# jfjlaros/HUMID

Hardware: AMD Instinct MI355X
Metric: reads/sec deduplicated, 10M PE150 UMI=8 d=1 (higher is better)
Workload: dtype u64; 1 GPU; 10000000 reads/GPU x 1 GPU (one shuffled read set of 10000000 reads, sliced by input order), PE150 UMI=8 in header -> 24-nt packed words (8+8+8), d=1, directional clustering; synthetic molecules=N/4, family 1+Geom(3), p_sub=1e-3, p_N=1e-4; reads_per_gpu=10000000, word_nt=24, distance=1, method=directional

## Files before the change

### humid_amd/_lib.py

```python
from __future__ import annotations

import ctypes as C
import os

_HERE = os.path.dirname(os.path.abspath(__file__))
SO_PATH = os.path.join(_HERE, "libhumid_hip.so")

u64p = C.POINTER(C.c_uint64)
u32p = C.POINTER(C.c_uint32)
u8p = C.POINTER(C.c_uint8)


class HumidSummary(C.Structure):
    _fields_ = [("total", C.c_uint64), ("usable", C.c_uint64), ("unique", C.c_uint64),
                ("clusters", C.c_uint64), ("edges", C.c_uint64), ("nonsingle", C.c_uint64),
                ("ms_count", C.c_float), ("ms_neighbours", C.c_float), ("ms_cluster", C.c_float),
                ("ms_map", C.c_float), ("ms_total", C.c_float), ("ms_h2d", C.c_float),
                ("ms_d2h", C.c_float), ("ms_k_insert", C.c_float), ("ms_k_pairs", C.c_float),
                ("ms_k_cluster", C.c_float), ("ms_k_map", C.c_float), ("ms_k_part", C.c_float),
                ("ms_k_unperm", C.c_float), ("count_mode_used", C.c_uint32)]

    def asdict(self):
        d = {k: getattr(self, k) for k, _ in self._fields_}
        d["records8"] = bool(d["count_mode_used"] >> 8)
# ... 209 lines not shown
                                    C.c_uint64, C.c_uint64, C.c_uint64, u64p, u64p]),
    "humid_stage_unique": (C.c_int, [C.c_void_p, C.POINTER(C.c_void_p), C.POINTER(C.c_void_p),
                                     C.POINTER(C.c_void_p)]),
    "humid_stage_graph": (C.c_int, [C.c_void_p, C.c_void_p, C.c_void_p, C.c_uint64, C.c_uint32,
                                    C.c_uint32, C.c_uint32, C.POINTER(C.c_void_p),
                                    C.POINTER(C.c_void_p), C.POINTER(HumidSummary)]),
    "humid_stage_map": (C.c_int, [C.c_void_p, C.c_void_p, C.c_void_p, C.c_uint64, C.c_void_p,
                                  C.c_void_p]),
    "humid_stage_count_dense": (C.c_int, [C.c_void_p, C.c_void_p, C.c_void_p, C.c_uint64, C.c_uint32,
                                          C.c_uint64, C.c_uint64, u64p, C.c_uint32, u64p, u64p, u64p]),
    "humid_stage_map_dense": (C.c_int, [C.c_void_p, C.c_void_p, C.c_void_p, C.POINTER(C.c_void_p), u64p]),
    "humid_stage_pairs": (C.c_int, [C.c_void_p, C.c_void_p, C.c_uint64, C.c_uint32, C.c_uint32,
                                    C.c_uint32, C.c_uint32, C.POINTER(C.c_void_p), u64p]),
    "humid_graph_split_info": (C.c_int, [C.c_void_p, C.POINTER(C.c_uint64), C.POINTER(C.c_uint64), u32p]),
    "humid_group_records_info": (C.c_int, [C.c_void_p, u32p, u32p]),
    "humid_get_run_roads": (C.c_int, [C.c_void_p, C.POINTER(HumidRunRoads)]),
    "humid_stage_kernel_ms": (C.c_int, [C.c_void_p, C.POINTER(C.c_float), C.POINTER(C.c_float), u32p]),
    "humid_stage_route_words": (C.c_int, [C.c_void_p, C.c_void_p, C.c_uint64, C.POINTER(C.c_void_p)]),
    "humid_stage_route": (C.c_int, [C.c_void_p, C.c_void_p, C.c_void_p, C.c_uint64, u64p, u64p, C.c_uint32, u64p,
                                    C.POINTER(C.c_void_p), C.POINTER(C.c_void_p)]),
    "humid_stage_route_check": (C.c_int, [C.c_void_p]),
    "humid_stage_exchange_ids": (C.c_int, [C.c_void_p, C.c_void_p, C.c_void_p, C.c_void_p, C.c_uint64,
                                           C.c_uint64, C.c_uint64, C.c_uint64, C.POINTER(C.c_void_p),
                                           C.POINTER(C.c_void_p)]),
    "humid_stage_plan_info": (C.c_int, [C.c_void_p, C.c_uint32, C.c_uint32, C.c_uint64, u32p, u32p]),
    "humid_stage_combo_route": (C.c_int, [C.c_void_p, C.c_void_p, C.c_void_p, C.c_uint64, C.c_uint64,
                                          C.c_uint32, C.c_uint32, C.c_uint64, C.c_uint32, C.c_uint32,
                                          C.POINTER(C.c_void_p), u64p]),
    "humid_stage_pairs_keyed": (C.c_int, [C.c_void_p, C.c_void_p, C.c_uint64, C.c_int, C.c_uint64,
                                          C.c_void_p, C.c_uint32, C.c_uint32, C.c_uint64, C.c_uint32,
# ... 66 lines not shown
```

### humid_amd/api.py

```python
from __future__ import annotations

import ctypes as C

import numpy as np

from . import _lib

DIRECTIONAL = 0
MAXIMUM = 1

BEST_LEAF, BEST_CLUSTER = 0, 1
NO_READ = 0xffffffff
NO_TILE = 0xffffffff
_BEST_SCOPES = {"leaf": BEST_LEAF, "cluster": BEST_CLUSTER, BEST_LEAF: BEST_LEAF, BEST_CLUSTER: BEST_CLUSTER}

STRAND_TOP, STRAND_BOTTOM, STRAND_NONE = 0, 1, 2

BC_FILTERED, BC_EXACT, BC_CORRECTED, BC_AMBIGUOUS, BC_UNMATCHED = range(5)

CELLS_TOP, CELLS_EXPECTED, CELLS_MIN_READS = 0, 1, 2


class HumidError(RuntimeError):
    def __init__(self, code, msg):
# ... 621 lines not shown
            self._check(self._lib.humid_get_leaf_groups(self._h, _vp(out["group"])))
        if getattr(self, "_keyed_summary", None) is self.summary:
            out["key"] = self.group_keys()[out["group"]] if u else np.zeros(0, np.uint64)
        return out

    def graph_split_info(self):
        a, b, f = C.c_uint64(), C.c_uint64(), C.c_uint32()
        self._check(self._lib.humid_graph_split_info(self._h, C.byref(a), C.byref(b), C.byref(f)))
        return dict(pairs_direct=a.value, pairs_graph=b.value, full_graph_built=f.value)

    def group_records_info(self):
        a, b = C.c_uint32(), C.c_uint32()
        self._check(self._lib.humid_group_records_info(self._h, C.byref(a), C.byref(b)))
        return dict(searched_on_records=a.value, orders_stored=b.value)

    def run_roads(self):
        r = _lib.HumidRunRoads()
        self._check(self._lib.humid_get_run_roads(self._h, C.byref(r)))
        return r.asdict()

    def adjacency(self):
        u = int(self.summary["unique"])
        e2 = 2 * int(self.summary["edges"])
        off = np.zeros(u + 1, np.uint32)
        idx = np.zeros(max(e2, 1), np.uint32)
        self._check(self._lib.humid_get_adjacency(self._h, _vp(off), _vp(idx)))
        return off, idx[:e2]

    def clusters(self):
        c = int(self.summary["clusters"])
# ... 218 lines not shown
```

### humid_amd/csrc/humid_hip.hip

```cpp
#include "pipeline.hip.h"
#include "passes.hip.h"

static std::string g_err;
extern "C" __attribute__((visibility("hidden"))) void humid_set_global_error(const char *text) { g_err = text ? text : ""; }

extern "C" {

uint32_t humid_abi_version(void) { return HUMID_ABI_VERSION; }

int humid_device_count(void) {
  int n = 0;
  if (hipGetDeviceCount(&n) != hipSuccess) return 0;
  return n;
}

const char *humid_last_error(const humid_ctx *ctx) { return ctx ? ctx->err.c_str() : g_err.c_str(); }

int humid_ctx_create(humid_ctx **out, int device, void *stream) {
  humid_ctx *c = nullptr;
  if (!out) return fail(nullptr, HUMID_E_INVALID, "out is null");
  *out = nullptr;
  int ndev = 0;
  hipError_t e = hipGetDeviceCount(&ndev);
  if (e != hipSuccess || ndev == 0)
// ... 146 lines not shown
  }
  if (strcmp(key, "group_buckets") == 0) {
    c->group_buckets = value != 0;
    return HUMID_OK;
  }
  if (strcmp(key, "fused_search") == 0) {
    c->fused_search = value != 0;
    return HUMID_OK;
  }
  if (strcmp(key, "pair_split") == 0) {
    c->pair_split = value != 0;
    return HUMID_OK;
  }
  if (strcmp(key, "group_records") == 0) {
    c->group_records = value != 0;
    return HUMID_OK;
  }
  if (strcmp(key, "padded_partition") == 0) {
    c->pt_padded = value != 0;
    return HUMID_OK;
  }
  if (strcmp(key, "force_comm") == 0) {
    c->force_comm = value != 0;
    return HUMID_OK;
  }
  if (strcmp(key, "bucket_walk") == 0) {
    if (value < 0 || value > (1 << 24)) return fail(c, HUMID_E_INVALID, "bucket_walk must be 0 (no limit) .. 2^24");
    c->walk_max = (u32)value;
    return HUMID_OK;
  }
// ... 239 lines not shown
int humid_graph_split_info(humid_ctx *c, uint64_t *pairs_direct, uint64_t *pairs_graph, uint32_t *full_graph_built) {
  if (!c) return fail(nullptr, HUMID_E_INVALID, "ctx is null");
  if (!state_has_leaves(c)) return fail(c, HUMID_E_STATE, "no completed dedup run / graph stage in this context");
  const bool split = c->cg_valid && c->cg_split;
  if (pairs_direct) *pairs_direct = split ? c->cg_iso : 0;
  if (pairs_graph) *pairs_graph = split ? c->cg_R : c->E;
  if (full_graph_built) *full_graph_built = (!split || c->cg_full) ? 1u : 0u;
  return HUMID_OK;
}

int humid_group_records_info(humid_ctx *c, uint32_t *searched_on_records, uint32_t *orders_stored) {
  if (!c) return fail(nullptr, HUMID_E_INVALID, "ctx is null");
  if (!state_has_leaves(c)) return fail(c, HUMID_E_STATE, "no completed dedup run / graph stage in this context");
  if (searched_on_records) *searched_on_records = c->cg_valid ? c->gr_rides : 0u;
  if (orders_stored) *orders_stored = c->cg_valid ? c->gr_orders : 0u;
  return HUMID_OK;
}

int humid_get_run_roads(humid_ctx *c, humid_run_roads *out) {
  if (!c) return fail(nullptr, HUMID_E_INVALID, "ctx is null");
  if (!out) return fail(c, HUMID_E_INVALID, "null argument");
  if (c->state.holds == CtxState::NOTHING) return fail(c, HUMID_E_STATE, "no completed run or stage call in this context");
  *out = c->roads;
  return HUMID_OK;
}

int humid_get_leaves(humid_ctx *c, uint64_t *word, uint32_t *count, uint32_t *first_read,
                     uint32_t *degree, uint32_t *cluster_id, uint8_t *is_max_leaf) {
  NEED_LEAVES();
  size_t U = (size_t)c->gU;
// ... 1167 lines not shown
```

### humid_amd/csrc/kernels_part8.hip.h

```cpp
#ifndef HUMID_KERNELS_PART8_HIP_H
#define HUMID_KERNELS_PART8_HIP_H

#include "common.hip.h"
#include "kernels_count.hip.h"
#include "kernels_part.hip.h"

#define P8_CAP2_LOG 10u
#define P8_CAP2 (1u << P8_CAP2_LOG)
#define P8_RPT (P8_CAP2 / 256u)

struct RecKey {
  u64 lo, scale;
  u32 z, kbits;
  u32 pow2;
  __host__ __device__ __forceinline__ u64 operator()(u64 w) const { return ((w - lo) * scale) >> z; }
  __device__ __forceinline__ u64 word(u64 k) const {
    if (pow2) return lo + k;
    const u64 x = k << z, q = x / scale;
    return lo + q + ((x - q * scale) ? 1u : 0u);
  }
};

struct Reads8 {
  const u64 *words;
// ... 70 lines not shown
    goff[threadIdx.x] = threadIdx.x * cap1 + (had < cap1 ? had : cap1);
    if (had + c > cap1) ctr[OVER] = 1;
  }
  PH(5);
#pragma unroll
  for (u32 q = 0; q < PT_IPT; q++)
    if (binrank[q] != NONE32) srec[loff[binrank[q] >> 16] + (binrank[q] & 0xffffu)] = rec[q];
  __syncthreads();
  PH(6);
  p8_write_bins(srec, loff, nb, p8_group(loff[nb], nb), out,
                [&](u32 bin, u32 k) -> u64 { return goff[bin] + k < (bin + 1) * cap1 ? (u64)goff[bin] + k : ~0ull; });
  PH(7);
  PH_END(1, 7, (blockIdx.x & 15u) == 3u);
}

static __global__ void __launch_bounds__(1024, 8)
k_p8_scatter2(const u64 *__restrict__ in, const u32 *__restrict__ tprefix, const u32 *__restrict__ cbase, u32 kbits, u32 d1,
              u32 d2, u32 ibits, u32 cap1, u32 *cursor2, u64 *__restrict__ out, ull *ctr) {
  HUMID_GUARD_LAST_VGPR();
  __shared__ u64 srec[PT_TILE];
  __shared__ u32 cnt[PT_MAXBINS], loff[PT_MAXBINS + 1], goff[PT_MAXBINS], room[PT_MAXBINS], wsum[8];
  __shared__ u32 s_c, s_beg, s_cnt;
  PH_DECL;
  PH(0);
  if (blockIdx.x >= tprefix[1u << d1]) return;
  const u32 nb = 1u << d2;
  if (threadIdx.x == 0) {
    u32 c, b, n;
    pt_tile_of(tprefix, cbase, 1u << d1, blockIdx.x, cap1, c, b, n);
    s_c = c; s_beg = b; s_cnt = n;
  }
  for (u32 b = threadIdx.x; b < nb; b += PT_THREADS) cnt[b] = 0;
  __syncthreads();
  PH(1);
  const u32 coarse = s_c, t_beg = s_beg, t_cnt = s_cnt;
  const u32 fshift = ibits + kbits - d1 - d2;
  u64 rec[PT_IPT];
  u32 binrank[PT_IPT];
#pragma unroll
  for (u32 q = 0; q < PT_IPT; q++) {
    const u32 j = threadIdx.x + q * PT_THREADS;
    binrank[q] = NONE32;
    if (j < t_cnt) rec[q] = in[t_beg + j];
  }
#pragma unroll
  for (u32 q = 0; q < PT_IPT; q++) {
    const u32 j = threadIdx.x + q * PT_THREADS;
    if (j < t_cnt) {
      const u32 bin = (u32)(rec[q] >> fshift) & (nb - 1);
      binrank[q] = bin << 16 | atomicAdd(&cnt[bin], 1u);
// ... 519 lines not shown
```

### humid_amd/csrc/pipeline.hip.h

```cpp
#ifndef HUMID_PIPELINE_HIP_H
#define HUMID_PIPELINE_HIP_H

#include <fcntl.h>
#include <sys/mman.h>
#include <sys/stat.h>
#include <unistd.h>

#include <atomic>
#include <cerrno>
#include <chrono>
#include <type_traits>
#include <utility>

#include "common.hip.h"
#include "prims.hip.h"
#include "kernels_count.hip.h"
#include "kernels_part.hip.h"
#include "kernels_part8.hip.h"
#include "kernels_graph.hip.h"
#include "kernels_cluster.hip.h"
#include "kernels_cgraph.hip.h"
#include "kernels_map.hip.h"
#include "kernels_xchg.hip.h"
#include "kernels_wide.hip.h"
// ... 127 lines not shown
  const u32 *ctr_x[3] = {nullptr, nullptr, nullptr};
  DBuf xo_gw, xo_gc;
  DBuf xo_regs, xo_inv;
  u64 xr_ecap = 0;
  DBuf xo_send, xo_int, xo_cross, xo_sel, xo_selall, xo_parent, xo_flag, xo_xroot, xo_xcbits, xo_xcblk, xo_xcid, xo_xcall, xo_ldeg, xo_cnt;
  DBuf pw_a, pw_ai, pw_b, pw_bi;
  DBuf p8_a, p8_b, p8_cur, p8_status;
  bool use_rec8 = true;
  bool last_rec8 = false;
  const u32 *rec_cursor2 = nullptr;
  DBuf pt_work, unperm_rec, route_tiles;
  bool group_buckets = true;
  bool fused_search = true;
  bool group_records = true;
  u32 gr_rides = 0, gr_orders = 0;
  bool pt_padded = true;
  bool use_tile_partition = true;
  bool last_part_tiled = false;
  int x_test_fail_after = -1, x_gathers = 0;
  bool x_hist_done = false, x_peer_failed = false;
  bool route_checked = true;
  const u32 *route_bad = nullptr;
  bool last_unperm_tiled = false;
  bool oc_valid = false, oc_fits = false;
  u32 oc_n = 0, oc_nt = 0;
  u64 oc_lo = 0, oc_scale = 0;
  u32 n_parts = 0;
  bool stage_map_timed = false;
  bool last_count_sorted = false;
  u32 g_wpr = 1;
// ... 166 lines not shown
  }
  __threadfence_system();
  __syncthreads();
  if (threadIdx.x == 0) { host[CTR_N] = seq; __threadfence_system(); }
}
static int read_counters_begin(humid_ctx *c, const u32 *extra32 = nullptr, const u32 *extra32b = nullptr, const u32 *extra32c = nullptr) {
  c->ctr_x[0] = extra32; c->ctr_x[1] = extra32b; c->ctr_x[2] = extra32c;
  if (c->h_ctr_dev && !c->no_poll) {
    const ull seq = ++c->ctr_seq;
    hipLaunchKernelGGL(k_publish_counters, dim3(1), dim3(64), 0, c->stream, (const ull *)c->d_ctr, extra32, extra32b,
                       (volatile ull *)c->h_ctr_dev, seq, extra32c);
    HIPCHK(hipGetLastError());
  }
  return HUMID_OK;
}
static int read_counters_end(humid_ctx *c) {
  const u32 *extra32 = c->ctr_x[0], *extra32b = c->ctr_x[1], *extra32c = c->ctr_x[2];
  if (c->h_ctr_dev && !c->no_poll) {
    const ull seq = c->ctr_seq;
    volatile ull *flag = (volatile ull *)&c->h_ctr[CTR_N];
    const auto t0 = std::chrono::steady_clock::now();
    u32 spins = 0;
    while (*flag != seq) {
      if ((++spins & 0xfffu) == 0) {
        if (hipStreamQuery(c->stream) != hipErrorNotReady) break;
        if (std::chrono::steady_clock::now() - t0 > std::chrono::seconds(30)) break;
      }
    }
    if (*flag == seq) { std::atomic_thread_fence(std::memory_order_acquire); return HUMID_OK; }
    HIPCHK(hipStreamSynchronize(c->stream));
    if (*flag == seq) return HUMID_OK;
    c->no_poll = true;
// ... 12 lines not shown
static int read_counters(humid_ctx *c, const u32 *extra32 = nullptr, const u32 *extra32b = nullptr, const u32 *extra32c = nullptr) {
  const int rc = read_counters_begin(c, extra32, extra32b, extra32c);
  return rc != HUMID_OK ? rc : read_counters_end(c);
}

#define TRY(...) do { int _rc = (__VA_ARGS__); if (_rc != HUMID_OK) return _rc; } while (0)

static int scan_total(humid_ctx *c, const u32 *in, u32 *out, u64 n, u64 *total) {
  TRY(exscan_u32(c, in, out, n + 1));
  HIPCHK(hipGetLastError());
  TRY(read_counters(c, out + n));
  *total = c->h_ctr[CTR_N - 1] & 0xffffffffull;
  return HUMID_OK;
}

static inline void state_reset(humid_ctx *c) { c->state = CtxState{}; c->roads = humid_run_roads{}; }
static inline void road_taken(humid_ctx *c, u8 road) {
  if (c->roads.n_events < HUMID_ROADS_MAX) c->roads.events[c->roads.n_events] = road;
  c->roads.n_events++;
}
static inline void state_begin_graph(humid_ctx *c) { const bool dense = c->state.dense; state_reset(c); c->state.dense = dense; }
static inline int state_publish(humid_ctx *c, CtxState::Holds holds) {
  const bool dense = holds == CtxState::STAGE_GRAPH && c->state.dense;
  c->state = CtxState{holds, holds == CtxState::RUN ? c->pass_kind : RUN_PLAIN, dense, false};
  return HUMID_OK;
}
static inline int state_publish_count(humid_ctx *c, bool dense) { state_publish(c, CtxState::COUNT); c->state.dense = dense; return HUMID_OK; }
static inline bool state_has_leaves(const humid_ctx *c) { return c->state.holds == CtxState::RUN || c->state.holds == CtxState::STAGE_GRAPH; }
static inline bool state_has_run(const humid_ctx *c) { return c->state.holds == CtxState::RUN; }
static inline bool state_dense_count(const humid_ctx *c) { return c->state.dense; }
static inline bool state_run_is(const humid_ctx *c, RunKind at_least) { return state_has_run(c) && c->state.kind >= at_least; }
// ... 109 lines not shown
    hipLaunchKernelGGL(k_cluster_trivial<true>, dim3(blocks_for(U)), dim3(256), 0, st, g.deg, g.parent, g.csize, U, g_cnt, g.off,
                       g.idx, g.cl_of, g.maxleaf, g.cl_size);
  else
    hipLaunchKernelGGL(k_cluster_trivial<false>, dim3(blocks_for(U)), dim3(256), 0, st, g.deg, g.parent, g.csize, U, g_cnt, g.off,
                       g.idx, g.cl_of, g.maxleaf, g.cl_size);
  if (M > 0) {
    const u64 small_cap = M / 3 + 1;
    if (late_m) TRY(read_counters_begin(c, nullptr, nullptr, late_m));
    if (method == HUMID_METHOD_MAXIMUM)
      hipLaunchKernelGGL(k_cluster_small_lds<true>, dim3(blocks_for(small_cap, 64)), dim3(64), 0, st, c->small_roots.as<u32>(),
                         (const ull *)c->d_ctr, g.parent, g.csize, U, g_cnt, g.off, g.idx, g.cl_of, g.maxleaf, g.cl_size);
    else
      hipLaunchKernelGGL(k_cluster_small_lds<false>, dim3(blocks_for(small_cap, 64)), dim3(64), 0, st, c->small_roots.as<u32>(),
                         (const ull *)c->d_ctr, g.parent, g.csize, U, g_cnt, g.off, g.idx, g.cl_of, g.maxleaf, g.cl_size);
    if (late_m) {
      TRY(read_counters_end(c));
      Mbig = c->h_ctr[CTR_MEMBERS];
      M = c->h_ctr[CTR_N - 3] & 0xffffffffull;
      U = (u32)M;
      if (late_m_out) *late_m_out = M;
    }
    if (Mbig > 0) {
      ENSURE(c->mk0, (size_t)Mbig * 8);
      ENSURE(c->mk1, (size_t)Mbig * 8);
      ENSURE(c->stk, (size_t)Mbig * 8);
      HIPCHK(hipMemsetAsync(&c->d_ctr[CTR_SPECIAL], 0, sizeof(ull), st));
      hipLaunchKernelGGL(k_member_keys, dim3(COMPACT_BLOCKS), dim3(256), 0, st, g.deg, g.parent, g.csize, U, c->mk0.as<u64>(), c->d_ctr);
      TRY(sort_keys<u64>(c, c->mk0.as<u64>(), c->mk1.as<u64>(), Mbig, 0, 32 + bits_for(U)));
      if (method == HUMID_METHOD_MAXIMUM) {
        hipLaunchKernelGGL(k_cluster_components<true>, dim3(blocks_for(Mbig, 64)), dim3(64), 0, st,
                           c->mk1.as<u64>(), (u32)Mbig, g_cnt, g.off, g.idx, g.cl_of, g.maxleaf, g.cl_size, c->stk.as<u32>());
// ... 311 lines not shown
    z.p[0] = cursor1; z.n[0] = PT_MAXBINS1 + n_parts;
    z.p[1] = (u32 *)c->d_ctr; z.n[1] = 2 * CTR_N;
    z.p[2] = (u32 *)(agg + n_parts); z.n[2] = 2;
    hipLaunchKernelGGL(k_zero_many, dim3(32), dim3(256), 0, st, z);
  }
  const bool check_range = !(range_lo == 0 && range_hi == ~0ull);
  const Reads8 src{d_words, d_filt, range_lo, range_hi, check_range ? 1u : 0u, rk};
  const u32 tiles1 = (N + PT_TILE - 1) / PT_TILE, tiles2 = tiles1 + nb1;
  static const bool s1_small = getenv("HUMID_S1_THREADS") ? atoi(getenv("HUMID_S1_THREADS")) == 512 : false;
  if (s1_small && nb1 <= 512)
    hipLaunchKernelGGL((k_p8_scatter1<Reads8, 512>), dim3((N + 4095) / 4096), dim3(512), 0, st, src, N, rk.kbits, d1, ibits, cap1, cursor1,
                       c->p8_a.as<u64>(), c->d_ctr);
  else
    hipLaunchKernelGGL((k_p8_scatter1<Reads8, 1024>), dim3(tiles1), dim3(1024), 0, st, src, N, rk.kbits, d1, ibits, cap1, cursor1,
                       c->p8_a.as<u64>(), c->d_ctr);
  hipLaunchKernelGGL(k_pt_scan1, dim3(1), dim3(1024), 0, st, (const u32 *)cursor1, d1, d2, cbase, tprefix, c->pbeg.as<u32>(),
                     c->ucount.as<u32>() + n_parts, cap1);
  if (c->kev_on) HIPCHK(hipEventRecord(c->kev[39], st));
  hipLaunchKernelGGL(k_p8_scatter2, dim3(tiles2), dim3(1024), 0, st, (const u64 *)c->p8_a.as<u64>(), (const u32 *)tprefix,
                     (const u32 *)cbase, rk.kbits, d1, d2, ibits, cap1, cursor2, c->p8_b.as<u64>(), c->d_ctr);
  if (c->kev_on) HIPCHK(hipEventRecord(c->kev[40], st));
  HIPCHK(hipEventRecord(c->kev[0], st));
  hipLaunchKernelGGL(k_dedup_rec, dim3(n_parts), dim3(256), 0, st, c->p8_b.as<u64>(), (const u32 *)cursor2, N, pb, d1, ibits, rk,
                     c->pad_word.as<u64>(), c->pad_cf.as<uint2>(), agg, c->d_ctr);
  HIPCHK(hipEventRecord(c->kev[1], st));
  TRY(exscan_in<u64>(c, PtrIn<u64>{agg}, abase, (u64)n_parts + 1));
  ENSURE(c->s_word, (size_t)(N + 1) * 8);
  ENSURE(c->s_slot, (size_t)(N + 1) * 4);
  ENSURE(c->s_cnt, (size_t)(N + 1) * 4);
  ENSURE(c->s_first, (size_t)(N + 1) * 4);
  hipLaunchKernelGGL(k_compact_padded8, dim3(blocks_for((u64)n_parts * 64)), dim3(256), 0, st, c->pad_word.as<u64>(),
                     c->pad_cf.as<uint2>(), (const u64 *)agg, (const u64 *)abase, n_parts, c->s_word.as<u64>(),
                     c->s_slot.as<u32>(), c->s_cnt.as<u32>(), c->s_first.as<u32>());
  if (!c->lean_events) HIPCHK(hipEventRecord(c->ev[1], st));
  HIPCHK(hipGetLastError());
  TRY(read_counters(c, (const u32 *)(abase + n_parts), (const u32 *)(abase + n_parts) + 1));
  if (getenv("HUMID_TRACE_COUNT"))
    fprintf(stderr, "[rec count] N %u pb %u kbits %u ibits %u cap1 %u special %llu overfull %llu unique %llu usable %llu\n", N, pb, rk.kbits,
            ibits, cap1, (ull)c->h_ctr[CTR_SPECIAL], (ull)c->h_ctr[CTR_OVERFULL], (ull)(c->h_ctr[CTR_N - 1] & 0xffffffffull), (ull)(c->h_ctr[CTR_N - 2] & 0xffffffffull));
  if (c->h_ctr[CTR_SPECIAL]) { c->pt_padded = false; road_taken(c, HUMID_ROAD_PART_PADDED_REDO); return HUMID_OK; }
  if (c->h_ctr[CTR_OVERFULL]) return HUMID_OK;
  c->last_count_lds = true;
  c->last_count_sorted = false;
  c->last_count_ordered = true;
  c->last_part_tiled = true;
  c->last_rec8 = true;
  c->rec_cursor2 = cursor2;
  c->n_parts = n_parts;
  const u32 U = (u32)(c->h_ctr[CTR_N - 1] & 0xffffffffull);
  s.usable = c->usable = c->h_ctr[CTR_N - 2] & 0xffffffffull;
  s.unique = c->U = U;
// ... 55 lines not shown
  if (c->kev_on) HIPCHK(hipEventRecord(c->kev[40], st));
  HIPCHK(hipEventRecord(c->kev[0], st));
  hipLaunchKernelGGL((k_dedup_wide_rec<9, 512, 0, WL_SMALL_LEN>), dim3(n_parts), dim3(256), 0, st, (const W2 *)c->pw_b.as<W2>(),
                     (const u32 *)c->pw_bi.as<u32>(), (const u32 *)cursor2, hbits, rk, N, pb, c->pad_word.as<W2>(), c->pad_cf.as<uint2>(),
                     agg, c->p8_b.as<u64>(), c->d_ctr);
  if (N > WL_SMALL_LEN)
    hipLaunchKernelGGL((k_dedup_wide_rec<10, 1024, WL_SMALL_LEN, WL_STAGE>), dim3(n_parts), dim3(256), 0, st,
                       (const W2 *)c->pw_b.as<W2>(), (const u32 *)c->pw_bi.as<u32>(), (const u32 *)cursor2, hbits, rk, N, pb,
                       c->pad_word.as<W2>(), c->pad_cf.as<uint2>(), agg, c->p8_b.as<u64>(), c->d_ctr);
  HIPCHK(hipEventRecord(c->kev[1], st));
  TRY(exscan_in<u64>(c, PtrIn<u64>{agg}, abase, (u64)n_parts + 1));
  ENSURE(c->s_word, (size_t)(N + 1) * 16);
  ENSURE(c->s_slot, (size_t)(N + 1) * 4);
  ENSURE(c->s_cnt, (size_t)(N + 1) * 4);
  ENSURE(c->s_first, (size_t)(N + 1) * 4);
  hipLaunchKernelGGL(k_compact_padded8_wide, dim3(blocks_for((u64)n_parts * 64)), dim3(256), 0, st, (const W2 *)c->pad_word.as<W2>(),
                     (const uint2 *)c->pad_cf.as<uint2>(), (const u64 *)agg, (const u64 *)abase, n_parts, c->s_word.as<W2>(),
                     c->s_slot.as<u32>(), c->s_cnt.as<u32>(), c->s_first.as<u32>());
  if (!c->lean_events) HIPCHK(hipEventRecord(c->ev[1], st));
  HIPCHK(hipGetLastError());
  TRY(read_counters(c, (const u32 *)(abase + n_parts), (const u32 *)(abase + n_parts) + 1));
  if (getenv("HUMID_TRACE_COUNT"))
    fprintf(stderr, "[rec count, wide] N %u pb %u kbits %u cap1 %u special %llu overfull %llu unique %llu usable %llu\n", N, pb, rk.kbits, cap1,
            (ull)c->h_ctr[CTR_SPECIAL], (ull)c->h_ctr[CTR_OVERFULL], (ull)(c->h_ctr[CTR_N - 1] & 0xffffffffull), (ull)(c->h_ctr[CTR_N - 2] & 0xffffffffull));
  if (c->h_ctr[CTR_SPECIAL] || c->h_ctr[CTR_OVERFULL]) return HUMID_OK;
  c->last_count_lds = true;
  c->last_count_sorted = false;
  c->last_count_ordered = true;
  c->last_part_tiled = true;
  c->last_rec8 = true;
  c->rec_cursor2 = cursor2;
  c->n_parts = n_parts;
  const u32 U = (u32)(c->h_ctr[CTR_N - 1] & 0xffffffffull);
  s.usable = c->usable = c->h_ctr[CTR_N - 2] & 0xffffffffull;
  s.unique = c->U = U;
  *done = true;
// ... 587 lines not shown
  const u32 *cnt_by_id;
  u32 n_ids;
  u64 pairs_bound;
  u32 *bits = nullptr;
  bool no_wait = false;
};
struct CgStatus {
  bool overflow = false;
  bool group_over = false;
  u64 wanted = 0, big_mask = 0, E = 0, M = 0, Mbig = 0;
};
static GraphArrays cg_arrays(humid_ctx *c) {
  return GraphArrays{c->cg_deg.as<u32>(), c->cg_parent.as<u32>(), c->cg_csize.as<u32>(), c->cg_off.as<u32>(), c->cg_idx.as<u32>(),
                     c->cg_cl_of.as<u32>(), c->cg_maxleaf.as<u32>(), c->cg_cl_size.as<u64>()};
}
static int cg_build(humid_ctx *c, CgSource &src, u32 method, CgStatus &out) {
  hipStream_t st = c->stream;
  u32 *bits = src.bits ? src.bits : c->cg_bits.as<u32>();
  const u32 n_words = (((src.n_ids + 31) / 32) + 7) & ~7u, n_blk = n_words / 8;
  const u64 pb = std::max<u64>(src.pairs_bound, 1);
  if (2 * pb + 2 > 0xffffffffull) return fail(c, HUMID_E_OVERFLOW, "too many neighbour pairs");
  const u32 Mb = (u32)std::min<u64>(src.n_ids, 2 * pb);
  ENSURE(c->cg_blk, ((size_t)n_blk + 1) * 4);
  ENSURE(c->cg_nodes, ((size_t)Mb + 1) * 4);
  ENSURE(c->cg_ncnt, ((size_t)Mb + 1) * 4);
  ENSURE(c->cg_deg, ((size_t)Mb + 2) * 4);
  ENSURE(c->cg_off, ((size_t)Mb + 2) * 4);
  ENSURE(c->cg_parent, ((size_t)Mb + 1) * 4);
  ENSURE(c->cg_csize, ((size_t)Mb + 1) * 4);
  ENSURE(c->cg_curs, ((size_t)Mb + 1) * 4);
  ENSURE(c->cg_idx, (size_t)(2 * pb + 1) * 4);
  ENSURE(c->cg_cl_of, ((size_t)Mb + 1) * 4);
  ENSURE(c->cg_maxleaf, ((size_t)Mb + 1) * 4);
  ENSURE(c->cg_cl_size, ((size_t)Mb + 1) * 8);
  ENSURE(c->small_roots, ((size_t)Mb / 3 + 2) * 4);
  ENSURE(c->small, 64);
  TRY(exscan_in<u32>(c, BitsBlockIn{bits, n_blk}, c->cg_blk.as<u32>(), (u64)n_blk + 1));
  const BitRank br{bits, c->cg_blk.as<u32>()};
  const u32 *m_dev = c->cg_blk.as<u32>() + n_blk;
  const GraphArrays g = cg_arrays(c);
  const u32 r_first = src.er.e ? 0u : ER_REGIONS;
  hipLaunchKernelGGL(k_nodes_init, dim3(blocks_for(n_words)), dim3(256), 0, st, br, n_words, src.cnt_by_id, c->cg_nodes.as<u32>(),
                     c->cg_ncnt.as<u32>(), g.deg, g.parent, g.csize, c->cg_curs.as<u32>(), n_blk);
  const bool by_count = (method & 1) == 0;
  if (src.segs) {
    const u32 n_all = src.segs->first[REC_SEGS];
    u32 n_max = 1;
    for (u32 q = 0; q < REC_SEGS; q++) n_max = std::max(n_max, src.segs->n[q]);
    ENSURE(c->cg_far, ((size_t)n_all + 1) * 8);
    hipLaunchKernelGGL(k_segs_relabel, dim3(std::min<u32>(blocks_for(n_max), 4096), REC_SEGS), dim3(256), 0, st, *src.segs, src.n_ids, br,
                       c->cg_far.as<u64>(), c->cg_ncnt.as<u32>(), g.deg, g.parent, by_count);
    src.er.far = c->cg_far.as<u64>();
    src.er.n_far = n_all;
  } else if (src.recs) {
    ENSURE(c->cg_far, ((size_t)src.n_recs + 1) * 8);
    if (src.n_recs)
      hipLaunchKernelGGL(k_records_relabel, dim3(blocks_for(src.n_recs)), dim3(256), 0, st, src.recs, src.n_recs, src.n_ids, br,
                         c->cg_far.as<u64>(), c->cg_ncnt.as<u32>(), g.deg, g.parent, by_count);
// ... 20 lines not shown
  else
    hipLaunchKernelGGL(k_cg_trivial<false>, dim3(tg), dim3(256), 0, st, (const u32 *)g.parent, (const u32 *)g.csize, m_dev,
                       (const u32 *)c->cg_ncnt.as<u32>(), (const u32 *)g.off, (const u32 *)g.idx, g.cl_of, g.maxleaf, g.cl_size, c->d_ctr,
                       c->small_roots.as<u32>());
  HIPCHK(hipGetLastError());
  if (src.no_wait) return HUMID_OK;
  TRY(read_counters(c, g.off + Mb, c->small.as<u32>(), m_dev));
  out.wanted = (c->h_ctr[CTR_N - 2] & 0xffffffffull) * ER_REGIONS;
  out.overflow = (c->h_ctr[CTR_EOVER] & 0xffffffffull) != 0;
  out.group_over = c->h_ctr[CTR_GOVER] != 0;
  out.big_mask = c->h_ctr[CTR_BIGMASK];
  out.E = (c->h_ctr[CTR_N - 1] & 0xffffffffull) / 2;
  out.M = c->h_ctr[CTR_N - 3] & 0xffffffffull;
  out.Mbig = c->h_ctr[CTR_MEMBERS];
  return HUMID_OK;
}
static int cg_cluster_rest(humid_ctx *c, u32 n_ids, u64 M, u64 Mbig, u32 method, const u32 *late_m = nullptr, bool fetch = false,
                           u64 *late_m_out = nullptr) {
  hipStream_t st = c->stream;
  const u32 n_words = (((n_ids + 31) / 32) + 7) & ~7u, n_blk = n_words / 8;
  const GraphArrays g = cg_arrays(c);
  ENSURE(c->cg_nblk, ((size_t)n_blk + 1) * 4);
  if (M > 0) TRY(cluster_kernels(c, g, c->cg_ncnt.as<u32>(), (u32)M, M, Mbig, method, true, fetch ? late_m : (const u32 *)nullptr, late_m_out));
  else if (c->kev_on) HIPCHK(hipEventRecord(c->kev[3], st));
  if (M > 0)
    hipLaunchKernelGGL(k_noncreator_bits, dim3(blocks_for(M)), dim3(256), 0, st, (const u32 *)g.cl_of, c->cg_nodes.as<u32>(), (u32)M,
                       c->cg_nbits.as<u32>(), late_m);
  TRY(exscan_in<u32>(c, BitsBlockIn{c->cg_nbits.as<u32>(), n_blk}, c->cg_nblk.as<u32>(), (u64)n_blk + 1));
  HIPCHK(hipGetLastError());
  return HUMID_OK;
// ... 108 lines not shown
    if (n_far)
      hipLaunchKernelGGL(k_mark_pairs, dim3(blocks_for(n_far)), dim3(256), 0, st, far, (u32)n_far, U, c->cg_bits.as<u32>(), bad, multi);
    if (split) {
      const u64 rest_cap = (u64)ER_REGIONS * er.cap_r + n_far;
      if (rest_cap > 0x7fffffffull) return fail(c, HUMID_E_OVERFLOW, "too many neighbour pairs");
      ENSURE(c->cg_rest, (size_t)(rest_cap + 1) * 8);
      const u32 gx = (u32)std::min<u64>(std::max<u64>(blocks_for(std::max<u64>(er.cap_r, er.n_far), SPLIT_PPT * 256), 1), 4096);
      u32 *sp = c->small.as<u32>();
      if (method == HUMID_METHOD_MAXIMUM)
        hipLaunchKernelGGL(k_pairs_split<true>, dim3(gx, ER_REGIONS + 1), dim3(256), 0, st, er, (const u32 *)multi, g_cnt, c->cg_pres.as<u32>(),
                           c->cg_nbits.as<u32>(), c->cg_rbits.as<u32>(), c->cg_rest.as<u64>(), (u32)rest_cap, U, sp);
      else
        hipLaunchKernelGGL(k_pairs_split<false>, dim3(gx, ER_REGIONS + 1), dim3(256), 0, st, er, (const u32 *)multi, g_cnt, c->cg_pres.as<u32>(),
                           c->cg_nbits.as<u32>(), c->cg_rbits.as<u32>(), c->cg_rest.as<u64>(), (u32)rest_cap, U, sp);
      HIPCHK(hipGetLastError());
      TRY(read_counters(c, sp + SPLIT_REST, sp + SPLIT_RMAX, sp + SPLIT_ALL));
      cgs.wanted = (c->h_ctr[CTR_N - 2] & 0xffffffffull) * ER_REGIONS;
      cgs.overflow = (c->h_ctr[CTR_EOVER] & 0xffffffffull) != 0;
      cgs.group_over = c->h_ctr[CTR_GOVER] != 0;
      cgs.big_mask = c->h_ctr[CTR_BIGMASK];
      R = c->h_ctr[CTR_N - 1] & 0xffffffffull;
      n_iso = (c->h_ctr[CTR_N - 3] & 0xffffffffull) - std::min<u64>(R, c->h_ctr[CTR_N - 3] & 0xffffffffull);
    } else {
      CgSource src;
      src.er = er; src.recs = nullptr; src.n_recs = 0; src.cnt_by_id = g_cnt; src.n_ids = U;
      src.pairs_bound = ecap + n_far;
      TRY(cg_build(c, src, method, cgs));
      er = src.er;
    }
    if (cgs.group_over) {
      c->gf_padded = false;
// ... 59 lines not shown
  }
  const u32 *late_m = nullptr;
  bool fetch = false;
  if (split) {
    c->cg_split = true;
    c->cg_method = method;
    c->cg_iso = n_iso; c->cg_R = R;
    E = n_iso + R;
    if (R > 0) {
      CgSource src;
      src.er.e = nullptr; src.er.cap_r = 0; src.er.cur = c->cg_cur.as<u32>(); src.er.far = c->cg_rest.as<u64>(); src.er.n_far = (u32)R;
      src.recs = nullptr; src.n_recs = 0; src.cnt_by_id = g_cnt; src.n_ids = U;
      src.pairs_bound = R;
      src.bits = c->cg_rbits.as<u32>();
      src.no_wait = true;
      TRY(cg_build(c, src, method, cgs));
      late_m = c->cg_blk.as<u32>() + n_blk;
      fetch = R >= SMALL_COMP;
      c->cg_m_late = !fetch;
      M = std::min<u64>(U, 2 * R);
      Mbig = 0;
    } else if (c->kev_on) HIPCHK(hipEventRecord(c->kev[2], st));
  }
  s.edges = c->E = E;
  if (!c->lean_events) HIPCHK(hipEventRecord(c->ev[2], st));
  u64 M_rest = 0;
  TRY(cg_cluster_rest(c, U, M, Mbig, method, late_m, fetch, &M_rest));
  if (split) M = 2 * n_iso + (fetch ? M_rest : 0);
  s.nonsingle = c->M = M;
  c->cg_M = split ? 0u : (u32)M;
  const GraphArrays g = cg_arrays(c);
// ... 13 lines not shown
  n_pair_segs_out = nseg < 8 ? nseg : 8;
  return HUMID_OK;
}

static int n_clusters_compact(humid_ctx *c, u32 U, u64 *out) {
  TRY(read_counters(c, c->cg_nblk.as<u32>() + c->cg_nblocks, c->cg_m_late ? c->cg_blk.as<u32>() + c->cg_nblocks : (const u32 *)nullptr));
  *out = (u64)U - (c->h_ctr[CTR_N - 1] & 0xffffffffull);
  if (c->cg_m_late) { c->M += c->h_ctr[CTR_N - 2] & 0xffffffffull; c->cg_m_late = false; }
  return HUMID_OK;
}

static int cg_build_full(humid_ctx *c) {
  hipStream_t st = c->stream;
  struct NoKernelEvents { humid_ctx *c; bool on; ~NoKernelEvents() { c->kev_on = on; } } quiet{c, c->kev_on};
  c->kev_on = false;
  {
    ZeroList z;
    memset(&z, 0, sizeof z);
    z.p[0] = (u32 *)&c->d_ctr[CTR_EDGES]; z.n[0] = 2 * (CTR_GOVER - CTR_EDGES + 1);
    hipLaunchKernelGGL(k_zero_many, dim3(1), dim3(256), 0, st, z);
  }
  CgSource src;
  src.er = c->cg_er; src.recs = nullptr; src.n_recs = 0; src.cnt_by_id = c->g_cnt; src.n_ids = c->gU;
  src.pairs_bound = c->cg_pairs_bound;
  CgStatus cgs;
  TRY(cg_build(c, src, c->cg_method, cgs));
  if (cgs.E != c->E) return fail(c, HUMID_E_INVALID, "internal: the full graph has %llu pairs, the run found %llu", (ull)cgs.E, (ull)c->E);
  if (cgs.M > 0) TRY(cluster_kernels(c, cg_arrays(c), c->cg_ncnt.as<u32>(), (u32)cgs.M, cgs.M, cgs.Mbig, c->cg_method, true));
  HIPCHK(hipStreamSynchronize(st));
  c->cg_M = (u32)cgs.M;
// ... 1151 lines not shown
```

### include/humid_hip.h

```cpp
#ifndef HUMID_HIP_H
#define HUMID_HIP_H

#include <stddef.h>
#include <stdint.h>

#ifdef __cplusplus
extern "C" {
#endif

#define HUMID_OK             0
#define HUMID_E_INVALID     -1
#define HUMID_E_UNSUPPORTED -2
#define HUMID_E_NOMEM       -3
#define HUMID_E_HIP         -4
#define HUMID_E_OVERFLOW    -5
#define HUMID_E_STATE       -6

#define HUMID_METHOD_DIRECTIONAL 0u
#define HUMID_METHOD_MAXIMUM     1u

#define HUMID_ABI_VERSION 5u

typedef struct humid_ctx humid_ctx;

// ... 319 lines not shown

int humid_stage_owned_results(humid_ctx *ctx, const uint32_t *d_local_cluster_id,
                              const uint8_t *d_local_is_max, const uint64_t *shard_begin,
                              uint32_t n_shards, const uint32_t **d_packed, uint64_t *counts);
int humid_stage_owner_perm(humid_ctx *ctx, const uint64_t *d_words, const uint8_t *d_filtered,
                           uint64_t n_reads, const uint64_t *range_lo, const uint64_t *range_hi,
                           uint32_t n_ranks, const uint32_t **d_perm, uint64_t *counts);
int humid_stage_owner_perm_wide(humid_ctx *ctx, const uint64_t *d_words, const uint8_t *d_filtered,
                                uint64_t n_reads, uint32_t word_nt, const uint64_t *range_lo, const uint64_t *range_hi,
                                uint32_t n_ranks, const uint32_t **d_perm, uint64_t *counts);
int humid_stage_scatter(humid_ctx *ctx, const uint32_t *d_perm, const uint32_t *d_packed,
                        uint64_t n_recv, uint64_t n_reads, uint32_t *d_cluster_id, uint8_t *d_keep);

int humid_graph_split_info(humid_ctx *ctx, uint64_t *pairs_direct, uint64_t *pairs_graph, uint32_t *full_graph_built);
int humid_group_records_info(humid_ctx *ctx, uint32_t *searched_on_records, uint32_t *orders_stored);
#define HUMID_ROAD_PART_PADDED_REDO 1
#define HUMID_ROAD_ORDERS_REDONE    2
#define HUMID_ROAD_REGIONS_REGROWN  3
#define HUMID_ROAD_FAR_TILES        4
#define HUMID_ROAD_CSR_TILES        5
#define HUMID_ROAD_JOIN_PIECES      6
#define HUMID_ROADS_MAX 32
typedef struct humid_run_roads {
  uint32_t n_events;
  uint32_t graph_attempts;
  uint8_t events[HUMID_ROADS_MAX];
} humid_run_roads;
int humid_get_run_roads(humid_ctx *ctx, humid_run_roads *out);
int humid_stage_kernel_ms(humid_ctx *ctx, float *ms_k_insert, float *ms_k_map, uint32_t *count_mode_used);
int humid_stage_route_words(humid_ctx *ctx, const uint64_t *d_words, uint64_t n_send,
// ... 58 lines not shown
```

Baseline: 18.06 billion reads/s.

## Overlap host counter waits with queued work and use static scatter tiles

Adds two default-on options. The first starts the host counter readback before the compact kernel, and before the graph front-end (block scan and node init) in the split path, so the host wait overlaps GPU work instead of stalling an idle queue. The second drops the single-block tile-prefix scan before the second scatter pass and launches a fixed grid in which each block derives its coarse bucket and offset from the cursor counts. That grid has many blocks that exit early and is sized by capacity rather than actual fill. The graph build is split into front and back halves to make the overlap possible.

```diff
diff --git a/humid_amd/_lib.py b/humid_amd/_lib.py
--- a/humid_amd/_lib.py
+++ b/humid_amd/_lib.py
@@ -247,6 +247,7 @@
                                     C.c_uint32, C.c_uint32, C.POINTER(C.c_void_p), u64p]),
     "humid_graph_split_info": (C.c_int, [C.c_void_p, C.POINTER(C.c_uint64), C.POINTER(C.c_uint64), u32p]),
     "humid_group_records_info": (C.c_int, [C.c_void_p, u32p, u32p]),
+    "humid_wait_overlap_info": (C.c_int, [C.c_void_p, u32p, u32p]),
     "humid_get_run_roads": (C.c_int, [C.c_void_p, C.POINTER(HumidRunRoads)]),
     "humid_stage_kernel_ms": (C.c_int, [C.c_void_p, C.POINTER(C.c_float), C.POINTER(C.c_float), u32p]),
     "humid_stage_route_words": (C.c_int, [C.c_void_p, C.c_void_p, C.c_uint64, C.POINTER(C.c_void_p)]),
diff --git a/humid_amd/api.py b/humid_amd/api.py
--- a/humid_amd/api.py
+++ b/humid_amd/api.py
@@ -659,6 +659,11 @@
         self._check(self._lib.humid_group_records_info(self._h, C.byref(a), C.byref(b)))
         return dict(searched_on_records=a.value, orders_stored=b.value)
 
+    def wait_overlap_info(self):
+        a, b = C.c_uint32(), C.c_uint32()
+        self._check(self._lib.humid_wait_overlap_info(self._h, C.byref(a), C.byref(b)))
+        return dict(host_waits=a.value, overlapped=b.value)
+
     def run_roads(self):
         r = _lib.HumidRunRoads()
         self._check(self._lib.humid_get_run_roads(self._h, C.byref(r)))
diff --git a/humid_amd/csrc/humid_hip.hip b/humid_amd/csrc/humid_hip.hip
--- a/humid_amd/csrc/humid_hip.hip
+++ b/humid_amd/csrc/humid_hip.hip
@@ -184,6 +184,14 @@
   }
   if (strcmp(key, "group_records") == 0) {
     c->group_records = value != 0;
+    return HUMID_OK;
+  }
+  if (strcmp(key, "overlap_waits") == 0) {
+    c->overlap_waits = value != 0;
+    return HUMID_OK;
+  }
+  if (strcmp(key, "static_tiles") == 0) {
+    c->static_tiles = value != 0;
     return HUMID_OK;
   }
   if (strcmp(key, "padded_partition") == 0) {
@@ -453,6 +461,14 @@
   if (!state_has_leaves(c)) return fail(c, HUMID_E_STATE, "no completed dedup run / graph stage in this context");
   if (searched_on_records) *searched_on_records = c->cg_valid ? c->gr_rides : 0u;
   if (orders_stored) *orders_stored = c->cg_valid ? c->gr_orders : 0u;
+  return HUMID_OK;
+}
+
+int humid_wait_overlap_info(humid_ctx *c, uint32_t *host_waits, uint32_t *overlapped) {
+  if (!c) return fail(nullptr, HUMID_E_INVALID, "ctx is null");
+  if (c->state.holds == CtxState::NOTHING) return fail(c, HUMID_E_STATE, "no completed run or stage call in this context");
+  if (host_waits) *host_waits = c->wo_waits;
+  if (overlapped) *overlapped = c->wo_overlapped;
   return HUMID_OK;
 }
 
diff --git a/humid_amd/csrc/kernels_part8.hip.h b/humid_amd/csrc/kernels_part8.hip.h
--- a/humid_amd/csrc/kernels_part8.hip.h
+++ b/humid_amd/csrc/kernels_part8.hip.h
@@ -108,6 +108,7 @@
   PH_END(1, 7, (blockIdx.x & 15u) == 3u);
 }
 
+template <bool STATIC>
 static __global__ void __launch_bounds__(1024, 8)
 k_p8_scatter2(const u64 *__restrict__ in, const u32 *__restrict__ tprefix, const u32 *__restrict__ cbase, u32 kbits, u32 d1,
               u32 d2, u32 ibits, u32 cap1, u32 *cursor2, u64 *__restrict__ out, ull *ctr) {
@@ -117,17 +118,30 @@
   __shared__ u32 s_c, s_beg, s_cnt;
   PH_DECL;
   PH(0);
-  if (blockIdx.x >= tprefix[1u << d1]) return;
   const u32 nb = 1u << d2;
-  if (threadIdx.x == 0) {
-    u32 c, b, n;
-    pt_tile_of(tprefix, cbase, 1u << d1, blockIdx.x, cap1, c, b, n);
-    s_c = c; s_beg = b; s_cnt = n;
-  }
-  for (u32 b = threadIdx.x; b < nb; b += PT_THREADS) cnt[b] = 0;
-  __syncthreads();
+  u32 coarse, t_beg, t_cnt;
+  if constexpr (STATIC) {
+    coarse = blockIdx.x & ((1u << d1) - 1u);
+    const u32 done = (blockIdx.x >> d1) * PT_TILE;
+    u32 fill = tprefix[coarse];
+    if (fill > cap1) fill = cap1;
+    if (done >= fill) return;
+    t_beg = coarse * cap1 + done;
+    t_cnt = fill - done < PT_TILE ? fill - done : PT_TILE;
+    for (u32 b = threadIdx.x; b < nb; b += PT_THREADS) cnt[b] = 0;
+    __syncthreads();
+  } else {
+    if (blockIdx.x >= tprefix[1u << d1]) return;
+    if (threadIdx.x == 0) {
+      u32 c, b, n;
+      pt_tile_of(tprefix, cbase, 1u << d1, blockIdx.x, cap1, c, b, n);
+      s_c = c; s_beg = b; s_cnt = n;
+    }
+    for (u32 b = threadIdx.x; b < nb; b += PT_THREADS) cnt[b] = 0;
+    __syncthreads();
+    coarse = s_c; t_beg = s_beg; t_cnt = s_cnt;
+  }
   PH(1);
-  const u32 coarse = s_c, t_beg = s_beg, t_cnt = s_cnt;
   const u32 fshift = ibits + kbits - d1 - d2;
   u64 rec[PT_IPT];
   u32 binrank[PT_IPT];
diff --git a/humid_amd/csrc/pipeline.hip.h b/humid_amd/csrc/pipeline.hip.h
--- a/humid_amd/csrc/pipeline.hip.h
+++ b/humid_amd/csrc/pipeline.hip.h
@@ -165,6 +165,9 @@
   bool fused_search = true;
   bool group_records = true;
   u32 gr_rides = 0, gr_orders = 0;
+  bool overlap_waits = true;
+  bool static_tiles = true;
+  u32 wo_waits = 0, wo_overlapped = 0;
   bool pt_padded = true;
   bool use_tile_partition = true;
   bool last_part_tiled = false;
@@ -361,8 +364,10 @@
   }
   return HUMID_OK;
 }
-static int read_counters_end(humid_ctx *c) {
+static int read_counters_end(humid_ctx *c, bool work_queued = false) {
   const u32 *extra32 = c->ctr_x[0], *extra32b = c->ctr_x[1], *extra32c = c->ctr_x[2];
+  c->wo_waits++;
+  if (work_queued) c->wo_overlapped++;
   if (c->h_ctr_dev && !c->no_poll) {
     const ull seq = c->ctr_seq;
     volatile ull *flag = (volatile ull *)&c->h_ctr[CTR_N];
@@ -405,7 +410,7 @@
   return HUMID_OK;
 }
 
-static inline void state_reset(humid_ctx *c) { c->state = CtxState{}; c->roads = humid_run_roads{}; }
+static inline void state_reset(humid_ctx *c) { c->state = CtxState{}; c->roads = humid_run_roads{}; c->wo_waits = c->wo_overlapped = 0; }
 static inline void road_taken(humid_ctx *c, u8 road) {
   if (c->roads.n_events < HUMID_ROADS_MAX) c->roads.events[c->roads.n_events] = road;
   c->roads.n_events++;
@@ -545,7 +550,7 @@
       hipLaunchKernelGGL(k_cluster_small_lds<false>, dim3(blocks_for(small_cap, 64)), dim3(64), 0, st, c->small_roots.as<u32>(),
                          (const ull *)c->d_ctr, g.parent, g.csize, U, g_cnt, g.off, g.idx, g.cl_of, g.maxleaf, g.cl_size);
     if (late_m) {
-      TRY(read_counters_end(c));
+      TRY(read_counters_end(c, true));
       Mbig = c->h_ctr[CTR_MEMBERS];
       M = c->h_ctr[CTR_N - 3] & 0xffffffffull;
       U = (u32)M;
@@ -887,11 +892,17 @@
   else
     hipLaunchKernelGGL((k_p8_scatter1<Reads8, 1024>), dim3(tiles1), dim3(1024), 0, st, src, N, rk.kbits, d1, ibits, cap1, cursor1,
                        c->p8_a.as<u64>(), c->d_ctr);
-  hipLaunchKernelGGL(k_pt_scan1, dim3(1), dim3(1024), 0, st, (const u32 *)cursor1, d1, d2, cbase, tprefix, c->pbeg.as<u32>(),
-                     c->ucount.as<u32>() + n_parts, cap1);
-  if (c->kev_on) HIPCHK(hipEventRecord(c->kev[39], st));
-  hipLaunchKernelGGL(k_p8_scatter2, dim3(tiles2), dim3(1024), 0, st, (const u64 *)c->p8_a.as<u64>(), (const u32 *)tprefix,
-                     (const u32 *)cbase, rk.kbits, d1, d2, ibits, cap1, cursor2, c->p8_b.as<u64>(), c->d_ctr);
+  if (c->static_tiles) {
+    if (c->kev_on) HIPCHK(hipEventRecord(c->kev[39], st));
+    hipLaunchKernelGGL(k_p8_scatter2<true>, dim3(nb1 * ((cap1 + PT_TILE - 1) / PT_TILE)), dim3(1024), 0, st, (const u64 *)c->p8_a.as<u64>(),
+                       (const u32 *)cursor1, (const u32 *)nullptr, rk.kbits, d1, d2, ibits, cap1, cursor2, c->p8_b.as<u64>(), c->d_ctr);
+  } else {
+    hipLaunchKernelGGL(k_pt_scan1, dim3(1), dim3(1024), 0, st, (const u32 *)cursor1, d1, d2, cbase, tprefix, c->pbeg.as<u32>(),
+                       c->ucount.as<u32>() + n_parts, cap1);
+    if (c->kev_on) HIPCHK(hipEventRecord(c->kev[39], st));
+    hipLaunchKernelGGL(k_p8_scatter2<false>, dim3(tiles2), dim3(1024), 0, st, (const u64 *)c->p8_a.as<u64>(), (const u32 *)tprefix,
+                       (const u32 *)cbase, rk.kbits, d1, d2, ibits, cap1, cursor2, c->p8_b.as<u64>(), c->d_ctr);
+  }
   if (c->kev_on) HIPCHK(hipEventRecord(c->kev[40], st));
   HIPCHK(hipEventRecord(c->kev[0], st));
   hipLaunchKernelGGL(k_dedup_rec, dim3(n_parts), dim3(256), 0, st, c->p8_b.as<u64>(), (const u32 *)cursor2, N, pb, d1, ibits, rk,
@@ -902,12 +913,15 @@
   ENSURE(c->s_slot, (size_t)(N + 1) * 4);
   ENSURE(c->s_cnt, (size_t)(N + 1) * 4);
   ENSURE(c->s_first, (size_t)(N + 1) * 4);
+  const bool early = c->overlap_waits;
+  if (early) TRY(read_counters_begin(c, (const u32 *)(abase + n_parts), (const u32 *)(abase + n_parts) + 1));
   hipLaunchKernelGGL(k_compact_padded8, dim3(blocks_for((u64)n_parts * 64)), dim3(256), 0, st, c->pad_word.as<u64>(),
                      c->pad_cf.as<uint2>(), (const u64 *)agg, (const u64 *)abase, n_parts, c->s_word.as<u64>(),
                      c->s_slot.as<u32>(), c->s_cnt.as<u32>(), c->s_first.as<u32>());
   if (!c->lean_events) HIPCHK(hipEventRecord(c->ev[1], st));
   HIPCHK(hipGetLastError());
-  TRY(read_counters(c, (const u32 *)(abase + n_parts), (const u32 *)(abase + n_parts) + 1));
+  if (early) TRY(read_counters_end(c, true));
+  else TRY(read_counters(c, (const u32 *)(abase + n_parts), (const u32 *)(abase + n_parts) + 1));
   if (getenv("HUMID_TRACE_COUNT"))
     fprintf(stderr, "[rec count] N %u pb %u kbits %u ibits %u cap1 %u special %llu overfull %llu unique %llu usable %llu\n", N, pb, rk.kbits,
             ibits, cap1, (ull)c->h_ctr[CTR_SPECIAL], (ull)c->h_ctr[CTR_OVERFULL], (ull)(c->h_ctr[CTR_N - 1] & 0xffffffffull), (ull)(c->h_ctr[CTR_N - 2] & 0xffffffffull));
@@ -993,12 +1007,15 @@
   ENSURE(c->s_slot, (size_t)(N + 1) * 4);
   ENSURE(c->s_cnt, (size_t)(N + 1) * 4);
   ENSURE(c->s_first, (size_t)(N + 1) * 4);
+  const bool early = c->overlap_waits;
+  if (early) TRY(read_counters_begin(c, (const u32 *)(abase + n_parts), (const u32 *)(abase + n_parts) + 1));
   hipLaunchKernelGGL(k_compact_padded8_wide, dim3(blocks_for((u64)n_parts * 64)), dim3(256), 0, st, (const W2 *)c->pad_word.as<W2>(),
                      (const uint2 *)c->pad_cf.as<uint2>(), (const u64 *)agg, (const u64 *)abase, n_parts, c->s_word.as<W2>(),
                      c->s_slot.as<u32>(), c->s_cnt.as<u32>(), c->s_first.as<u32>());
   if (!c->lean_events) HIPCHK(hipEventRecord(c->ev[1], st));
   HIPCHK(hipGetLastError());
-  TRY(read_counters(c, (const u32 *)(abase + n_parts), (const u32 *)(abase + n_parts) + 1));
+  if (early) TRY(read_counters_end(c, true));
+  else TRY(read_counters(c, (const u32 *)(abase + n_parts), (const u32 *)(abase + n_parts) + 1));
   if (getenv("HUMID_TRACE_COUNT"))
     fprintf(stderr, "[rec count, wide] N %u pb %u kbits %u cap1 %u special %llu overfull %llu unique %llu usable %llu\n", N, pb, rk.kbits, cap1,
             (ull)c->h_ctr[CTR_SPECIAL], (ull)c->h_ctr[CTR_OVERFULL], (ull)(c->h_ctr[CTR_N - 1] & 0xffffffffull), (ull)(c->h_ctr[CTR_N - 2] & 0xffffffffull));
@@ -1616,34 +1633,43 @@
   return GraphArrays{c->cg_deg.as<u32>(), c->cg_parent.as<u32>(), c->cg_csize.as<u32>(), c->cg_off.as<u32>(), c->cg_idx.as<u32>(),
                      c->cg_cl_of.as<u32>(), c->cg_maxleaf.as<u32>(), c->cg_cl_size.as<u64>()};
 }
-static int cg_build(humid_ctx *c, CgSource &src, u32 method, CgStatus &out) {
+static int cg_build_front(humid_ctx *c, const u32 *bits, u32 n_ids, const u32 *cnt_by_id, u64 nodes_bound) {
+  hipStream_t st = c->stream;
+  const u32 n_words = (((n_ids + 31) / 32) + 7) & ~7u, n_blk = n_words / 8;
+  const size_t Mb = (size_t)std::min<u64>(n_ids, nodes_bound);
+  ENSURE(c->cg_blk, ((size_t)n_blk + 1) * 4);
+  ENSURE(c->cg_nodes, (Mb + 1) * 4);
+  ENSURE(c->cg_ncnt, (Mb + 1) * 4);
+  ENSURE(c->cg_deg, (Mb + 2) * 4);
+  ENSURE(c->cg_parent, (Mb + 1) * 4);
+  ENSURE(c->cg_csize, (Mb + 1) * 4);
+  ENSURE(c->cg_curs, (Mb + 1) * 4);
+  TRY(exscan_in<u32>(c, BitsBlockIn{bits, n_blk}, c->cg_blk.as<u32>(), (u64)n_blk + 1));
+  const BitRank br{bits, c->cg_blk.as<u32>()};
+  const GraphArrays g = cg_arrays(c);
+  hipLaunchKernelGGL(k_nodes_init, dim3(blocks_for(n_words)), dim3(256), 0, st, br, n_words, cnt_by_id, c->cg_nodes.as<u32>(),
+                     c->cg_ncnt.as<u32>(), g.deg, g.parent, g.csize, c->cg_curs.as<u32>(), n_blk);
+  HIPCHK(hipGetLastError());
+  return HUMID_OK;
+}
+static int cg_build_back(humid_ctx *c, CgSource &src, u32 method, CgStatus &out) {
   hipStream_t st = c->stream;
   u32 *bits = src.bits ? src.bits : c->cg_bits.as<u32>();
   const u32 n_words = (((src.n_ids + 31) / 32) + 7) & ~7u, n_blk = n_words / 8;
   const u64 pb = std::max<u64>(src.pairs_bound, 1);
   if (2 * pb + 2 > 0xffffffffull) return fail(c, HUMID_E_OVERFLOW, "too many neighbour pairs");
   const u32 Mb = (u32)std::min<u64>(src.n_ids, 2 * pb);
-  ENSURE(c->cg_blk, ((size_t)n_blk + 1) * 4);
-  ENSURE(c->cg_nodes, ((size_t)Mb + 1) * 4);
-  ENSURE(c->cg_ncnt, ((size_t)Mb + 1) * 4);
-  ENSURE(c->cg_deg, ((size_t)Mb + 2) * 4);
   ENSURE(c->cg_off, ((size_t)Mb + 2) * 4);
-  ENSURE(c->cg_parent, ((size_t)Mb + 1) * 4);
-  ENSURE(c->cg_csize, ((size_t)Mb + 1) * 4);
-  ENSURE(c->cg_curs, ((size_t)Mb + 1) * 4);
   ENSURE(c->cg_idx, (size_t)(2 * pb + 1) * 4);
   ENSURE(c->cg_cl_of, ((size_t)Mb + 1) * 4);
   ENSURE(c->cg_maxleaf, ((size_t)Mb + 1) * 4);
   ENSURE(c->cg_cl_size, ((size_t)Mb + 1) * 8);
   ENSURE(c->small_roots, ((size_t)Mb / 3 + 2) * 4);
   ENSURE(c->small, 64);
-  TRY(exscan_in<u32>(c, BitsBlockIn{bits, n_blk}, c->cg_blk.as<u32>(), (u64)n_blk + 1));
   const BitRank br{bits, c->cg_blk.as<u32>()};
   const u32 *m_dev = c->cg_blk.as<u32>() + n_blk;
   const GraphArrays g = cg_arrays(c);
   const u32 r_first = src.er.e ? 0u : ER_REGIONS;
-  hipLaunchKernelGGL(k_nodes_init, dim3(blocks_for(n_words)), dim3(256), 0, st, br, n_words, src.cnt_by_id, c->cg_nodes.as<u32>(),
-                     c->cg_ncnt.as<u32>(), g.deg, g.parent, g.csize, c->cg_curs.as<u32>(), n_blk);
   const bool by_count = (method & 1) == 0;
   if (src.segs) {
     const u32 n_all = src.segs->first[REC_SEGS];
@@ -1694,6 +1720,12 @@
   out.M = c->h_ctr[CTR_N - 3] & 0xffffffffull;
   out.Mbig = c->h_ctr[CTR_MEMBERS];
   return HUMID_OK;
+}
+static int cg_build(humid_ctx *c, CgSource &src, u32 method, CgStatus &out) {
+  const u64 pb = std::max<u64>(src.pairs_bound, 1);
+  if (2 * pb + 2 > 0xffffffffull) return fail(c, HUMID_E_OVERFLOW, "too many neighbour pairs");
+  TRY(cg_build_front(c, src.bits ? src.bits : c->cg_bits.as<u32>(), src.n_ids, src.cnt_by_id, 2 * pb));
+  return cg_build_back(c, src, method, out);
 }
 static int cg_cluster_rest(humid_ctx *c, u32 n_ids, u64 M, u64 Mbig, u32 method, const u32 *late_m = nullptr, bool fetch = false,
                            u64 *late_m_out = nullptr) {
@@ -1832,7 +1864,12 @@
         hipLaunchKernelGGL(k_pairs_split<false>, dim3(gx, ER_REGIONS + 1), dim3(256), 0, st, er, (const u32 *)multi, g_cnt, c->cg_pres.as<u32>(),
                            c->cg_nbits.as<u32>(), c->cg_rbits.as<u32>(), c->cg_rest.as<u64>(), (u32)rest_cap, U, sp);
       HIPCHK(hipGetLastError());
-      TRY(read_counters(c, sp + SPLIT_REST, sp + SPLIT_RMAX, sp + SPLIT_ALL));
+      if (c->overlap_waits) {
+        TRY(read_counters_begin(c, sp + SPLIT_REST, sp + SPLIT_RMAX, sp + SPLIT_ALL));
+        TRY(cg_build_front(c, c->cg_rbits.as<u32>(), U, g_cnt, 2 * rest_cap));
+        TRY(read_counters_end(c, true));
+      } else
+        TRY(read_counters(c, sp + SPLIT_REST, sp + SPLIT_RMAX, sp + SPLIT_ALL));
       cgs.wanted = (c->h_ctr[CTR_N - 2] & 0xffffffffull) * ER_REGIONS;
       cgs.overflow = (c->h_ctr[CTR_EOVER] & 0xffffffffull) != 0;
       cgs.group_over = c->h_ctr[CTR_GOVER] != 0;
@@ -1922,7 +1959,8 @@
       src.pairs_bound = R;
       src.bits = c->cg_rbits.as<u32>();
       src.no_wait = true;
-      TRY(cg_build(c, src, method, cgs));
+      if (c->overlap_waits) TRY(cg_build_back(c, src, method, cgs));
+      else TRY(cg_build(c, src, method, cgs));
       late_m = c->cg_blk.as<u32>() + n_blk;
       fetch = R >= SMALL_COMP;
       c->cg_m_late = !fetch;
@@ -1966,6 +2004,7 @@
   hipStream_t st = c->stream;
   struct NoKernelEvents { humid_ctx *c; bool on; ~NoKernelEvents() { c->kev_on = on; } } quiet{c, c->kev_on};
   c->kev_on = false;
+  struct RunsWaits { humid_ctx *c; u32 w, o; ~RunsWaits() { c->wo_waits = w; c->wo_overlapped = o; } } waits{c, c->wo_waits, c->wo_overlapped};
   {
     ZeroList z;
     memset(&z, 0, sizeof z);
diff --git a/include/humid_hip.h b/include/humid_hip.h
--- a/include/humid_hip.h
+++ b/include/humid_hip.h
@@ -357,6 +357,7 @@
 
 int humid_graph_split_info(humid_ctx *ctx, uint64_t *pairs_direct, uint64_t *pairs_graph, uint32_t *full_graph_built);
 int humid_group_records_info(humid_ctx *ctx, uint32_t *searched_on_records, uint32_t *orders_stored);
+int humid_wait_overlap_info(humid_ctx *ctx, uint32_t *host_waits, uint32_t *overlapped);
 #define HUMID_ROAD_PART_PADDED_REDO 1
 #define HUMID_ROAD_ORDERS_REDONE    2
 #define HUMID_ROAD_REGIONS_REGROWN  3
```

Measured after the change: 18.41 billion reads/s, median of 6. 1.02x the previous value.
